# PeihaoChen/WS-MGMap

Hardware: AMD Instinct MI355X
Metric: policy steps/sec (fwd+bwd), CMA batch=8 seq=64 (higher is better)
Workload: dtype bf16

## Files before the change

ws-mgmap_amd/csrc/wsmg_conv_win.hip:

```cpp
#include <stdlib.h>

#include "wsmg_common.h"

namespace {

typedef __bf16 bf16_t;
typedef short bf16x8 __attribute__((ext_vector_type(8)));
typedef unsigned int u32x4 __attribute__((ext_vector_type(4)));

struct WinArgs {
  const bf16_t* x;
  const bf16_t* w;
  const float* bias;
  bf16_t* y;
  int B, H, W, OH, OW, tiles_y, tiles_x, relu;
  unsigned x_bytes, w_bytes;
  double* stats;
  int nslab;
};

__device__ __forceinline__ int xcd_swizzle(int bid, int nb) {
  const int q = nb >> 3, r = nb & 7, x = bid & 7;
  return x * q + (x < r ? x : r) + (bid >> 3);
}
__device__ __forceinline__ __amdgpu_buffer_rsrc_t make_rsrc(const void* p, unsigned bytes) {
  return __builtin_amdgcn_make_buffer_rsrc(const_cast<void*>(p), 0, (int)bytes, 0x00020000);
}
__device__ __forceinline__ u32x4 buf_load16(__amdgpu_buffer_rsrc_t r, int byte_off) {
  return __builtin_amdgcn_raw_buffer_load_b128(r, byte_off, 0, 0);
}
__device__ __forceinline__ unsigned short f2bf_bits(float f) {
  bf16_t b = (bf16_t)f;
  return __builtin_bit_cast(unsigned short, b);
}

template <int K, int S, int P, int TH, int TW>
__global__ __launch_bounds__(256) void conv_win_fwd_kernel(WinArgs a) {
  constexpr int CI = 64, CO = 64;
  constexpr int WR = (TH - 1) * S + K;
  constexpr int WC = (TW - 1) * S + K;
  constexpr int PC = WC / S;
  constexpr int PITCH = 144;
  constexpr int WIN_BYTES = WR * S * PC * PITCH;
  constexpr int BT_BYTES = CO * PITCH;
  constexpr int CHUNKS = WR * WC * 8;
  static_assert(WC % S == 0 && CHUNKS % 256 == 0 && TH * TW <= 128 && CI == 64, "tile geometry");
  extern __shared__ __attribute__((aligned(16))) unsigned char lds[];
  unsigned char* win = lds;
  unsigned char* bt = lds + WIN_BYTES;

  const int tid = threadIdx.x, lane = tid & 63, wave = tid >> 6;
  const int tpi = a.tiles_y * a.tiles_x;
  const int ntiles = a.B * tpi;
  const int per = (ntiles + (int)gridDim.x - 1) / (int)gridDim.x;
  const int first = xcd_swizzle(blockIdx.x, gridDim.x) * per;
  double st_s[2] = {0.0, 0.0}, st_q[2] = {0.0, 0.0};
  for (int logical = first; logical < first + per && logical < ntiles; ++logical) {
  const int b = logical / tpi, t = logical - b * tpi;
  const int oy0 = (t / a.tiles_x) * TH, ox0 = (t % a.tiles_x) * TW;
  const int iy0 = oy0 * S - P, ix0 = ox0 * S - P;
  const __amdgpu_buffer_rsrc_t xr = make_rsrc(a.x, a.x_bytes), wr_ = make_rsrc(a.w, a.w_bytes);

  const int bco = tid >> 3, bch = tid & 7;
  auto wload = [&](int tap, u32x4& p0, u32x4& p1) {
    p0 = buf_load16(wr_, ((bco * K * K + tap) * CI) * 2 + bch * 16);
    p1 = buf_load16(wr_, (((bco + 32) * K * K + tap) * CI) * 2 + bch * 16);
  };
  auto wstore = [&](int buf, const u32x4& p0, const u32x4& p1) {
    *reinterpret_cast<u32x4*>(bt + buf * BT_BYTES + bco * PITCH + bch * 16) = p0;
    *reinterpret_cast<u32x4*>(bt + buf * BT_BYTES + (bco + 32) * PITCH + bch * 16) = p1;
  };
  constexpr int RING = 7;
  u32x4 ring[RING][2];
#pragma unroll
  for (int tp = 0; tp < RING; ++tp) wload(tp, ring[tp][0], ring[tp][1]);
  constexpr int PER = CHUNKS / 256;
#pragma unroll
  for (int j0 = 0; j0 < PER; j0 += 14) {
    u32x4 v[14];
    int dst[14];
#pragma unroll
    for (int j = 0; j < 14; ++j) {
      const int c = tid + 256 * (j0 + j);
      const int pix = c >> 3, ch = c & 7;
      const int wr = pix / WC, wc = pix - wr * WC;
      const int iy = iy0 + wr, ix = ix0 + wc;
      const bool ok = iy >= 0 && iy < a.H && ix >= 0 && ix < a.W;
      const int off = ok ? (((b * a.H + iy) * a.W + ix) * CI) * 2 + ch * 16 : (int)0x80000000;
      v[j] = buf_load16(xr, off);
      dst[j] = ((wr * S + (wc % S)) * PC + wc / S) * PITCH + ch * 16;
    }
#pragma unroll
    for (int j = 0; j < 14; ++j) *reinterpret_cast<u32x4*>(win + dst[j]) = v[j];
  }
  wstore(0, ring[0][0], ring[0][1]);
  wstore(1, ring[1][0], ring[1][1]);
  wload(RING, ring[0][0], ring[0][1]);
  wload(RING + 1, ring[1][0], ring[1][1]);
  __syncthreads();

  const int r = lane & 31, h = lane >> 5;
  const int q = wave * 32 + r;
  const int qc = q < TH * TW ? q : TH * TW - 1;
  const int ty = qc / TW, tx = qc - ty * TW;
  const unsigned char* a_base = win + ((ty * S * S) * PC + tx) * PITCH + h * 16;
  const unsigned char* b_base = bt + r * PITCH + h * 16;
  f32x16 acc[2];
#pragma unroll
  for (int f = 0; f < 2; ++f)
#pragma unroll
    for (int g = 0; g < 16; ++g) acc[f][g] = 0.f;

  struct Frag { bf16x8 a[4], b0[4], b1[4]; };
  auto fload = [&](int tap, Frag& fr) {
    const int ky = tap / K, kx = tap % K;
    const unsigned char* ap = a_base + ((ky * S + (kx % S)) * PC + kx / S) * PITCH;
    const unsigned char* bp = b_base + (tap % 3) * BT_BYTES;
#pragma unroll
    for (int kc = 0; kc < 4; ++kc) {
      fr.a[kc] = *reinterpret_cast<const bf16x8*>(ap + kc * 32);
      fr.b0[kc] = *reinterpret_cast<const bf16x8*>(bp + kc * 32);
      fr.b1[kc] = *reinterpret_cast<const bf16x8*>(bp + 32 * PITCH + kc * 32);
    }
  };
  Frag cur, nxt;
  fload(0, cur);
#pragma unroll
  for (int tap = 0; tap < K * K; ++tap) {
    if (tap + 2 < K * K) {
      wstore((tap + 2) % 3, ring[(tap + 2) % RING][0], ring[(tap + 2) % RING][1]);
      if (tap + 2 + RING < K * K) wload(tap + 2 + RING, ring[(tap + 2) % RING][0], ring[(tap + 2) % RING][1]);
    }
    __builtin_amdgcn_sched_barrier(0);
    if (tap + 1 < K * K) fload(tap + 1, nxt);
#pragma unroll
    for (int kc = 0; kc < 4; ++kc) {
      acc[0] = __builtin_amdgcn_mfma_f32_32x32x16_bf16(cur.a[kc], cur.b0[kc], acc[0], 0, 0, 0);
      acc[1] = __builtin_amdgcn_mfma_f32_32x32x16_bf16(cur.a[kc], cur.b1[kc], acc[1], 0, 0, 0);
    }
#pragma unroll
    for (int i = 0; i < 4; ++i) {
      __builtin_amdgcn_sched_group_barrier(0x008, 1, 0);
      __builtin_amdgcn_sched_group_barrier(0x100, 2, 0);
      __builtin_amdgcn_sched_group_barrier(0x008, 1, 0);
      __builtin_amdgcn_sched_group_barrier(0x100, 1, 0);
    }
    __builtin_amdgcn_sched_barrier(0);
    if (tap + 1 < K * K) {
      if (tap + 2 < K * K) asm volatile("s_waitcnt lgkmcnt(12)\n\ts_barrier" ::: "memory");
      else asm volatile("s_barrier" ::: "memory");
      cur = nxt;
    }
  }

  asm volatile("s_waitcnt lgkmcnt(0)\n\ts_barrier" ::: "memory");
  unsigned okmask = 0;
  if (a.stats) {
#pragma unroll
    for (int g = 0; g < 16; ++g) {
      const int qq = wave * 32 + (g & 3) + 8 * (g >> 2) + 4 * h;
      const bool ok = qq < TH * TW && oy0 + qq / TW < a.OH && ox0 + qq % TW < a.OW;
      okmask |= ok ? 1u << g : 0u;
    }
  }
#pragma unroll
  for (int f = 0; f < 2; ++f) {
    const int co = 32 * f + r;
    const float bv = a.bias ? a.bias[co] : 0.f;
    float sv = 0.f, qv = 0.f;
#pragma unroll
    for (int g = 0; g < 16; ++g) {
      const int row = (g & 3) + 8 * (g >> 2) + 4 * h;
      float v = acc[f][g] + bv;
      if (a.relu) v = v > 0.f ? v : 0.f;
      const unsigned short o = f2bf_bits(v);
      *reinterpret_cast<unsigned short*>(win + (wave * 32 + row) * PITCH + co * 2) = o;
      const float vr = (okmask >> g) & 1u ? __uint_as_float((unsigned)o << 16) : 0.f;
      sv += vr;
      qv = fmaf(vr, vr, qv);
    }
    st_s[f] += (double)sv;
    st_q[f] += (double)qv;
  }
  __syncthreads();
#pragma unroll
  for (int j = 0; j < 4; ++j) {
    const int c = tid + 256 * j;
    const int qq = c >> 3, ch = c & 7;
    if (qq >= TH * TW) continue;
    const int oy = oy0 + qq / TW, ox = ox0 + qq % TW;
    if (oy >= a.OH || ox >= a.OW) continue;
    const u32x4 v = *reinterpret_cast<const u32x4*>(win + qq * PITCH + ch * 16);
    *reinterpret_cast<u32x4*>(reinterpret_cast<unsigned char*>(a.y) + (((size_t)(b * a.OH + oy) * a.OW + ox) * CO) * 2 + ch * 16) = v;
  }
  __syncthreads();
  }
  if (a.stats) {
    const int r = threadIdx.x & 31, h = (threadIdx.x >> 5) & 1;
#pragma unroll
    for (int f = 0; f < 2; ++f) {
      const double s2 = st_s[f] + __shfl_xor(st_s[f], 32, 64), q2 = st_q[f] + __shfl_xor(st_q[f], 32, 64);
      if (h == 0) {
        double* st = a.stats + (size_t)(blockIdx.x % a.nslab) * 2 * CO + 32 * f + r;
        atomicAdd(st, s2);
        atomicAdd(st + CO, q2);
      }
    }
  }
}

}

int wsmg_conv_win_fwd_bf16(const void* x, const void* w_ohwi, const float* bias, void* y, int relu, double* stats, int nslab, int B,
                           int H, int W, int Cin, int Cout, int KH, int KW, int stride, int pad, int OH, int OW, hipStream_t s) {
  if (Cin != 64 || Cout != 64 || KH != 8 || KW != 8 || stride != 2 || pad != 3) return WSMG_EINVAL;
  if ((size_t)B * H * W * 128 >= (1ull << 31)) return WSMG_EINVAL;
  constexpr int TH = 5, TW = 25;
  WinArgs a{(const bf16_t*)x, (const bf16_t*)w_ohwi, bias, (bf16_t*)y, B, H, W, OH, OW, (OH + TH - 1) / TH, (OW + TW - 1) / TW, relu,
            (unsigned)((size_t)B * H * W * 128), (unsigned)(64u * 8 * 8 * 64 * 2), stats, nslab};
  auto kern = conv_win_fwd_kernel<8, 2, 3, TH, TW>;
  constexpr int LDS = (((TH - 1) * 2 + 8) * 2 * (((TW - 1) * 2 + 8) / 2) + 3 * 64) * 144;
  static bool attr = false;
  if (!attr) {
    hipError_t e = hipFuncSetAttribute(reinterpret_cast<const void*>(kern), hipFuncAttributeMaxDynamicSharedMemorySize, LDS);
    if (e != hipSuccess) return (int)e;
    attr = true;
  }
  int ntiles = B * a.tiles_y * a.tiles_x, grid = ntiles < 256 ? ntiles : 256;
  hipLaunchKernelGGL(kern, dim3((unsigned)grid), dim3(256), LDS, s, a);
  WSMG_RETURN_LAUNCH();
}
```

Before: 52300.

## Prefetch next tile's input window into registers during current tile's MFMA loop

Restructures the persistent conv tile loop so the input window for the next tile is loaded into registers while the current tile's tap loop runs, then written to LDS at the start of the next iteration. The weight ring preload is also reissued at the end of each tile, and bias is hoisted out of the loop. This hides the global-load latency of the window fill behind MFMA work. The cost is much higher register pressure (32 extra 16-byte vectors per thread), which may cause spills or lower occupancy.

New measurement: 52600, median of 6. Within noise of the previous version (+0.6%).

```diff
diff --git a/ws-mgmap_amd/csrc/wsmg_conv_win.hip b/ws-mgmap_amd/csrc/wsmg_conv_win.hip
--- a/ws-mgmap_amd/csrc/wsmg_conv_win.hip
+++ b/ws-mgmap_amd/csrc/wsmg_conv_win.hip
@@ -3,6 +3,13 @@
 #include "wsmg_common.h"
 
 namespace {
+
+#ifndef WSMG_PF_T0
+#define WSMG_PF_T0 0
+#endif
+#ifndef WSMG_PF_N
+#define WSMG_PF_N 1
+#endif
 
 typedef __bf16 bf16_t;
 typedef short bf16x8 __attribute__((ext_vector_type(8)));
@@ -34,7 +41,7 @@
   return __builtin_bit_cast(unsigned short, b);
 }
 
-template <int K, int S, int P, int TH, int TW>
+template <int K, int S, int P, int TH, int TW, int PF_T0, int PF_N>
 __global__ __launch_bounds__(256) void conv_win_fwd_kernel(WinArgs a) {
   constexpr int CI = 64, CO = 64;
   constexpr int WR = (TH - 1) * S + K;
@@ -43,8 +50,7 @@
   constexpr int PITCH = 144;
   constexpr int WIN_BYTES = WR * S * PC * PITCH;
   constexpr int BT_BYTES = CO * PITCH;
-  constexpr int CHUNKS = WR * WC * 8;
-  static_assert(WC % S == 0 && CHUNKS % 256 == 0 && TH * TW <= 128 && CI == 64, "tile geometry");
+  static_assert(WC % S == 0 && TH * TW <= 128 && CI == 64, "tile geometry");
   extern __shared__ __attribute__((aligned(16))) unsigned char lds[];
   unsigned char* win = lds;
   unsigned char* bt = lds + WIN_BYTES;
@@ -55,10 +61,7 @@
   const int per = (ntiles + (int)gridDim.x - 1) / (int)gridDim.x;
   const int first = xcd_swizzle(blockIdx.x, gridDim.x) * per;
   double st_s[2] = {0.0, 0.0}, st_q[2] = {0.0, 0.0};
-  for (int logical = first; logical < first + per && logical < ntiles; ++logical) {
-  const int b = logical / tpi, t = logical - b * tpi;
-  const int oy0 = (t / a.tiles_x) * TH, ox0 = (t % a.tiles_x) * TW;
-  const int iy0 = oy0 * S - P, ix0 = ox0 * S - P;
+  const int last = first + per < ntiles ? first + per : ntiles;
   const __amdgpu_buffer_rsrc_t xr = make_rsrc(a.x, a.x_bytes), wr_ = make_rsrc(a.w, a.w_bytes);
 
   const int bco = tid >> 3, bch = tid & 7;
@@ -70,34 +73,57 @@
     *reinterpret_cast<u32x4*>(bt + buf * BT_BYTES + bco * PITCH + bch * 16) = p0;
     *reinterpret_cast<u32x4*>(bt + buf * BT_BYTES + (bco + 32) * PITCH + bch * 16) = p1;
   };
+  constexpr int PER = 2 * WR;
+  static_assert(WC > 32 && WC <= 64 && ((WC - 32) * 8) % 64 == 0, "two column pieces per thread and row");
+  static_assert(PER % PF_N == 0 && PER / PF_N <= K * K, "the prefetch fits the tap loop");
+  constexpr unsigned OOB = 0x80000000u;
+  const int wc0 = tid >> 3, pch = tid & 7;
+  const bool has1 = tid < (WC - 32) * 8;
+  const int xl0 = ((wc0 % S) * PC + wc0 / S) * PITCH + pch * 16;
+  constexpr int XL1 = (32 / S) * PITCH, XROW = S * PC * PITCH;
+  auto win_columns = [&](int logical, unsigned& cb0, unsigned& cb1, int& iy0, int& row0) {
+    const bool live = logical < last;
+    const int b = logical / tpi, t = logical - b * tpi;
+    const int c0 = (t % a.tiles_x) * TW * S - P + wc0, c1 = c0 + 32;
+    cb0 = live && (unsigned)c0 < (unsigned)a.W ? (unsigned)(c0 * CI * 2 + pch * 16) : OOB;
+    cb1 = live && has1 && (unsigned)c1 < (unsigned)a.W ? (unsigned)(c1 * CI * 2 + pch * 16) : OOB;
+    iy0 = (t / a.tiles_x) * TH * S - P;
+    row0 = b * a.H;
+  };
+  auto win_load = [&](int p, unsigned cb0, unsigned cb1, int iy0, int row0) {
+    const int iy = iy0 + (p >> 1);
+    const unsigned base = (unsigned)((row0 + iy) * a.W) * (CI * 2);
+    return buf_load16(xr, (int)((unsigned)iy < (unsigned)a.H ? base + ((p & 1) ? cb1 : cb0) : OOB));
+  };
   constexpr int RING = 7;
   u32x4 ring[RING][2];
+  u32x4 pre[PER];
+  unsigned cb0, cb1;
+  int wiy0, wrow0;
+  win_columns(first, cb0, cb1, wiy0, wrow0);
+#pragma unroll
+  for (int p = 0; p < PER; ++p) pre[p] = win_load(p, cb0, cb1, wiy0, wrow0);
 #pragma unroll
   for (int tp = 0; tp < RING; ++tp) wload(tp, ring[tp][0], ring[tp][1]);
-  constexpr int PER = CHUNKS / 256;
-#pragma unroll
-  for (int j0 = 0; j0 < PER; j0 += 14) {
-    u32x4 v[14];
-    int dst[14];
-#pragma unroll
-    for (int j = 0; j < 14; ++j) {
-      const int c = tid + 256 * (j0 + j);
-      const int pix = c >> 3, ch = c & 7;
-      const int wr = pix / WC, wc = pix - wr * WC;
-      const int iy = iy0 + wr, ix = ix0 + wc;
-      const bool ok = iy >= 0 && iy < a.H && ix >= 0 && ix < a.W;
-      const int off = ok ? (((b * a.H + iy) * a.W + ix) * CI) * 2 + ch * 16 : (int)0x80000000;
-      v[j] = buf_load16(xr, off);
-      dst[j] = ((wr * S + (wc % S)) * PC + wc / S) * PITCH + ch * 16;
-    }
-#pragma unroll
-    for (int j = 0; j < 14; ++j) *reinterpret_cast<u32x4*>(win + dst[j]) = v[j];
+  float bv[2];
+#pragma unroll
+  for (int f = 0; f < 2; ++f) bv[f] = a.bias ? a.bias[32 * f + (lane & 31)] : 0.f;
+
+  for (int logical = first; logical < last; ++logical) {
+  const int b = logical / tpi, t = logical - b * tpi;
+  const int oy0 = (t / a.tiles_x) * TH, ox0 = (t % a.tiles_x) * TW;
+
+#pragma unroll
+  for (int wr = 0; wr < WR; ++wr) {
+    *reinterpret_cast<u32x4*>(win + wr * XROW + xl0) = pre[2 * wr];
+    if (has1) *reinterpret_cast<u32x4*>(win + wr * XROW + xl0 + XL1) = pre[2 * wr + 1];
   }
   wstore(0, ring[0][0], ring[0][1]);
   wstore(1, ring[1][0], ring[1][1]);
   wload(RING, ring[0][0], ring[0][1]);
   wload(RING + 1, ring[1][0], ring[1][1]);
-  __syncthreads();
+  asm volatile("s_waitcnt lgkmcnt(0)\n\ts_barrier" ::: "memory");
+  win_columns(logical + 1, cb0, cb1, wiy0, wrow0);
 
   const int r = lane & 31, h = lane >> 5;
   const int q = wave * 32 + r;
@@ -131,6 +157,10 @@
       wstore((tap + 2) % 3, ring[(tap + 2) % RING][0], ring[(tap + 2) % RING][1]);
       if (tap + 2 + RING < K * K) wload(tap + 2 + RING, ring[(tap + 2) % RING][0], ring[(tap + 2) % RING][1]);
     }
+    if (tap >= PF_T0 && tap < PF_T0 + PER / PF_N) {
+#pragma unroll
+      for (int k = 0; k < PF_N; ++k) pre[(tap - PF_T0) * PF_N + k] = win_load((tap - PF_T0) * PF_N + k, cb0, cb1, wiy0, wrow0);
+    }
     __builtin_amdgcn_sched_barrier(0);
     if (tap + 1 < K * K) fload(tap + 1, nxt);
 #pragma unroll
@@ -153,6 +183,8 @@
     }
   }
 
+#pragma unroll
+  for (int tp = 0; tp < RING; ++tp) wload(tp, ring[tp][0], ring[tp][1]);
   asm volatile("s_waitcnt lgkmcnt(0)\n\ts_barrier" ::: "memory");
   unsigned okmask = 0;
   if (a.stats) {
@@ -166,12 +198,11 @@
 #pragma unroll
   for (int f = 0; f < 2; ++f) {
     const int co = 32 * f + r;
-    const float bv = a.bias ? a.bias[co] : 0.f;
     float sv = 0.f, qv = 0.f;
 #pragma unroll
     for (int g = 0; g < 16; ++g) {
       const int row = (g & 3) + 8 * (g >> 2) + 4 * h;
-      float v = acc[f][g] + bv;
+      float v = acc[f][g] + bv[f];
       if (a.relu) v = v > 0.f ? v : 0.f;
       const unsigned short o = f2bf_bits(v);
       *reinterpret_cast<unsigned short*>(win + (wave * 32 + row) * PITCH + co * 2) = o;
@@ -182,7 +213,7 @@
     st_s[f] += (double)sv;
     st_q[f] += (double)qv;
   }
-  __syncthreads();
+  asm volatile("s_waitcnt lgkmcnt(0)\n\ts_barrier" ::: "memory");
 #pragma unroll
   for (int j = 0; j < 4; ++j) {
     const int c = tid + 256 * j;
@@ -193,7 +224,7 @@
     const u32x4 v = *reinterpret_cast<const u32x4*>(win + qq * PITCH + ch * 16);
     *reinterpret_cast<u32x4*>(reinterpret_cast<unsigned char*>(a.y) + (((size_t)(b * a.OH + oy) * a.OW + ox) * CO) * 2 + ch * 16) = v;
   }
-  __syncthreads();
+  asm volatile("s_waitcnt lgkmcnt(0)\n\ts_barrier" ::: "memory");
   }
   if (a.stats) {
     const int r = threadIdx.x & 31, h = (threadIdx.x >> 5) & 1;
@@ -218,7 +249,7 @@
   constexpr int TH = 5, TW = 25;
   WinArgs a{(const bf16_t*)x, (const bf16_t*)w_ohwi, bias, (bf16_t*)y, B, H, W, OH, OW, (OH + TH - 1) / TH, (OW + TW - 1) / TW, relu,
             (unsigned)((size_t)B * H * W * 128), (unsigned)(64u * 8 * 8 * 64 * 2), stats, nslab};
-  auto kern = conv_win_fwd_kernel<8, 2, 3, TH, TW>;
+  auto kern = conv_win_fwd_kernel<8, 2, 3, TH, TW, WSMG_PF_T0, WSMG_PF_N>;
   constexpr int LDS = (((TH - 1) * 2 + 8) * 2 * (((TW - 1) * 2 + 8) / 2) + 3 * 64) * 144;
   static bool attr = false;
   if (!attr) {
```
